# nkargas/Gen2-UHF-RFID-Reader

Measured on AMD Instinct MI355X. Metric: I/Q Msamples/s through matched_filter->gate->tag_decoder (+ EPC decodes/s), 40 kHz FM0, higher is better.
Workload: dtype f32; 1 GPU; configs[1]: batch of 1024 noise-replicas per GPU of the 71-round file_source_test stand-in trace, FM0 40 kHz BLF @ 2 Msps (1076066 raw I/Q samples each, sigma=0.002), generated and resident in HBM; streams_per_gpu=1024, hbm_bytes_traces=8815132672, parallelism=traces sharded per GPU, no collective

## Files before the change

gen2-uhf-rfid-reader_amd/csrc/rfid_capi.hip:

```cpp
#include <hip/hip_runtime.h>

#include <cmath>
#include <ctime>
#include <pthread.h>
#include <cstdio>
#include <cstdlib>
#include <cstring>
#include <deque>
#include <initializer_list>
#include <map>
#include <memory>
#include <new>
#include <vector>

#include "rfid_host_math.h"
#include "rfid_kernels.hpp"
#include "rfid_inventory.hpp"
#include "rfid_tracks.hpp"
#include "rfid_quality.hpp"
#include "rfid_repair.hpp"
#include "rfid_mi355x.h"
#include "rfid_gen2_host.h"
#define LS2_LAUNCH(kernel, gx, gy, block, args) \
  hipLaunchKernelGGL(rfidk::kernel, dim3((unsigned)(gx), (unsigned)(gy)), dim3((unsigned)(block)), 0, ls2_stream, args)
// ... 1689 lines not shown
  if (!c || !ms) return RFID_ERR_INVALID;
  return stage_ms(c, c->rep, ms);
}

int rfid_repair_window(rfid_ctx *c, const rfid_cf32 *gated, const rfid_decode_result *res, rfid_repair *out) {
  if (!c || !gated || !res || !out) return RFID_ERR_INVALID;
  if (res->type != RFID_DECODE_EPC) return fail(c, RFID_ERR_INVALID, "rfid_repair_window: not the result of an EPC window");
  HIPCHK(c, hipSetDevice(c->device));
  const size_t sz_w = up256(sizeof(float2) * (size_t)EPC_WIN), sz_r = up256(sizeof(rfid_decode_result));
  { int r = grow(c, c->rep_one, sz_w + sz_r + sizeof(rfid_repair)); if (r) return r; }
  char *b = (char *)c->rep_one.p;
  HIPCHK(c, hipMemcpyAsync(b, gated, sizeof(float2) * (size_t)EPC_WIN, hipMemcpyHostToDevice, c->stream));
  HIPCHK(c, hipMemcpyAsync(b + sz_w, res, sizeof(*res), hipMemcpyHostToDevice, c->stream));
  hipLaunchKernelGGL(repair_one_kernel, dim3(1), dim3(64), 0, c->stream, (const float2 *)b, (const rfid_decode_result *)(b + sz_w),
                     (rfid_repair *)(b + sz_w + sz_r));
  HIPCHK(c, hipGetLastError());
  HIPCHK(c, hipMemcpyAsync(out, b + sz_w + sz_r, sizeof(*out), hipMemcpyDeviceToHost, c->stream));
  HIPCHK(c, hipStreamSynchronize(c->stream));
  return RFID_OK;
}

}

namespace {

int pass_long_stream(rfid_ctx *c, const void *d_raw, int64_t raw_stride, int64_t n_raw, const void *d_lens, int want_scores) {
  HIPCHK(c, hipSetDevice(c->device));
  { int rj = join_tails(c); if (rj) return rj; }
  const int64_t n_out = n_raw / DECIM;
  const int64_t tiles = (n_out + MF_TILE - 1) / MF_TILE;
  int rc, enq = 0;
  bool ahead = false;
  if (raw_stride >= 2) {
    c->d_lens = (const int64_t *)d_lens;
    c->last_n_raw = n_raw;
    c->n_chunks_last = 0;
    ahead = c->alt.d_y != nullptr && c->ls2_ws_alt.p != nullptr && !c->alt_have && (c->knobs.overlap != 0);
    if (ahead && (rc = y_take_ahead(c))) return rc;
    HIPCHK_T(c, ev_mark(c, EV_MF_BEGIN, c->stream));
    HIPCHK_T(c, ev_mark(c, EV_MF_END, c->stream));
    LsOpts lo;
    lo.raw = d_raw; lo.raw_stride = raw_stride; lo.ahead = ahead;
    if ((rc = ls_enqueue(c, n_out, lo, &enq))) { c->y_touched = true; return rc; }
    if (!enq && ahead) {
      y_give_back(c);
      ahead = lo.ahead = false;
      if ((rc = ls_enqueue(c, n_out, lo, &enq))) return rc;
    }
  }
  if (enq) {
    c->fused_last = 2;
    MfFallbackArgs f;
    f.m = mf_args(c, d_raw, raw_stride, n_raw);
    f.skip_if = &c->d_ls2_ctl->ok; f.n_tiles = tiles;
    if ((rc = launch_mf_rows(c, c->stream, f, (tiles < 4096) ? tiles : 4096)) || (rc = rfid_batch_gate_impl(c, &c->d_ls2_ctl->ok)) ||
        (rc = rfid_batch_decode(c, want_scores)) || (rc = rfid_batch_stats(c))) { c->y_touched = true; return rc; }
    return y_pass_done(c, ahead);
  }
  c->y_touched = true;
  if ((rc = batch_mf_on(c, c->stream, d_raw, raw_stride, n_raw, d_lens))) return rc;
  LsOpts lo;
  if ((rc = ls_enqueue(c, n_out, lo, &enq))) return rc;
  if ((rc = rfid_batch_gate_impl(c, enq ? &c->d_ls2_ctl->ok : nullptr))) return rc;
  if ((rc = rfid_batch_decode(c, want_scores))) return rc;
  return rfid_batch_stats(c);
}

int pass_fused(rfid_ctx *c, const void *d_raw, int64_t raw_stride, int64_t n_raw, const void *d_lens, int want_scores) {
  HIPCHK(c, hipSetDevice(c->device));
  c->d_lens = (const int64_t *)d_lens;
  c->last_n_raw = n_raw;
  c->n_chunks_last = 0;
  const bool overlap = c->alt_have && !want_scores;
  { int rj = overlap ? set_take_next(c) : join_tails(c); if (rj) return rj; }
  HIPCHK(c, ev_mark(c, EV_MF_BEGIN, c->stream));
  HIPCHK(c, ev_mark(c, EV_MF_END, c->stream));
  HIPCHK(c, hipMemsetAsync(c->d_gstate, 0, sizeof(GateState) * (size_t)c->B, c->stream));
  HIPCHK(c, hipMemsetAsync(c->cur.d_flat_count, 0, 2 * sizeof(int), c->stream));
  GateArgs g = gate_args(c, n_raw / DECIM);
  g.y_w = c->cur.d_y;
  g.raw = (const float2 *)d_raw; g.raw_stride = raw_stride; g.n_raw = n_raw;
  g.raw_vec_ok = rows_vec_ok(d_raw, raw_stride);
  g.single_step = c->knobs.front_single_step;
  hipLaunchKernelGGL(front_end_fused_kernel, gate_grid(c), dim3(GATE_THREADS), 0, c->stream, g);
  HIPCHK(c, hipGetLastError());
  HIPCHK(c, ev_mark(c, EV_GATE_END, c->stream));
  c->fused_last = 1;
  if (overlap) return set_tails_on_stream2(c);
  int rc = rfid_batch_decode(c, want_scores);
  if (rc) return rc;
  return rfid_batch_stats(c);
}

int pass_chunked(rfid_ctx *c, const void *d_raw, int64_t raw_stride, int64_t n_raw, const void *d_lens, int want_scores) {
  const int nch = c->knobs.front_chunks;
  const int64_t tiles = (n_raw / DECIM + MF_TILE - 1) / MF_TILE;
  HIPCHK(c, hipSetDevice(c->device));
  { int rj = join_tails(c); if (rj) return rj; }
  if (!c->ev_mf[0]) {
    for (int i = 0; i <= rfid_ctx::MAX_CHUNKS; ++i) HIPCHK(c, hipEventCreate(&c->ev_mf[i]));
    for (int i = 0; i < 2 * rfid_ctx::MAX_CHUNKS; ++i) HIPCHK(c, hipEventCreate(&c->ev_gate[i]));
  }
  c->d_lens = (const int64_t *)d_lens;
  c->last_n_raw = n_raw;
  const int64_t tiles_per_chunk = (tiles + nch - 1) / nch;
  HIPCHK(c, hipEventRecord(c->ev_pass, c->stream));
  HIPCHK(c, hipStreamWaitEvent(c->stream2, c->ev_pass, 0));
  HIPCHK(c, hipMemsetAsync(c->d_gstate, 0, sizeof(GateState) * (size_t)c->B, c->stream2));
  HIPCHK(c, hipMemsetAsync(c->cur.d_flat_count, 0, 2 * sizeof(int), c->stream2));
  MfArgs m = mf_args(c, d_raw, raw_stride, n_raw);
  GateArgs g = gate_args(c, n_raw / DECIM);
  HIPCHK(c, ev_mark(c, EV_MF_BEGIN, c->stream));
  HIPCHK(c, hipEventRecord(c->ev_mf[0], c->stream));
  int used = 0;
  for (int k = 0; k < nch; ++k) {
    const int64_t t0 = (int64_t)k * tiles_per_chunk;
    if (t0 >= tiles) break;
    const int64_t tn = (t0 + tiles_per_chunk <= tiles) ? tiles_per_chunk : (tiles - t0);
    m.tile0 = t0;
    { int r = launch_mf_rows(c, c->stream, m, tn); if (r) return r; }
    HIPCHK(c, hipEventRecord(c->ev_mf[k + 1], c->stream));
    HIPCHK(c, hipStreamWaitEvent(c->stream2, c->ev_mf[k + 1], 0));
    g.pos0 = t0 * MF_TILE; g.chunk_len = tn * MF_TILE;
    HIPCHK(c, hipEventRecord(c->ev_gate[2 * k], c->stream2));
    hipLaunchKernelGGL(gate_scan_kernel, gate_grid(c), dim3(GATE_THREADS), 0, c->stream2, g);
    HIPCHK(c, hipGetLastError());
    HIPCHK(c, hipEventRecord(c->ev_gate[2 * k + 1], c->stream2));
    used = k + 1;
  }
  c->n_chunks_last = used;
  HIPCHK(c, hipEventRecord(c->ev_front_end, c->stream2));
  HIPCHK(c, hipStreamWaitEvent(c->stream, c->ev_front_end, 0));
  c->ev_valid[EV_MF_END] = false;
  HIPCHK(c, ev_mark(c, EV_GATE_END, c->stream));
  int rc = rfid_batch_decode(c, want_scores);
  if (rc) return rc;
  return rfid_batch_stats(c);
}

}

extern "C" {

int rfid_batch_process(rfid_ctx *c, const void *d_raw, int64_t raw_stride, int64_t n_raw, const void *d_lens,
                       int want_scores) {
  if (!c || !d_raw || n_raw < 0 || raw_stride < n_raw) return RFID_ERR_INVALID;
  if (!c->B) return RFID_ERR_STATE;
  if (n_raw > c->max_raw) return RFID_ERR_CAPACITY;
  ls_note_last_pass(c);
  const int64_t n_out = n_raw / DECIM;
  const int64_t tiles = (n_out + MF_TILE - 1) / MF_TILE;
  const int nch = c->knobs.front_chunks;
  if (nch < 2 && ls_applicable(c, c->B, n_out)) return pass_long_stream(c, d_raw, raw_stride, n_raw, d_lens, want_scores);
  c->d_ls2_ctl = nullptr;
  c->y_touched = true;
  if (nch < 2 && raw_stride >= 2 && !c->knobs.front_unfused) return pass_fused(c, d_raw, raw_stride, n_raw, d_lens, want_scores);
  c->fused_last = 0;
  if (tiles < 4 * (int64_t)nch || nch < 2) {
    int rc = rfid_batch_mf(c, d_raw, raw_stride, n_raw, d_lens);
    if (rc) return rc;
    if ((rc = rfid_batch_gate(c))) return rc;
    if ((rc = rfid_batch_decode(c, want_scores))) return rc;
    return rfid_batch_stats(c);
  }
  return pass_chunked(c, d_raw, raw_stride, n_raw, d_lens, want_scores);
}

// ... 605 lines not shown
```

gen2-uhf-rfid-reader_amd/csrc/rfid_kernels.hpp:

```cpp
#pragma once
#include <rfid_device_env.h>
#include "rfid_mi355x.h"

namespace rfidk {

constexpr int DECIM = 5;
constexpr int NTAPS = 25;
constexpr int WIN_LEN = 100;
constexpr int DC_LEN = 48;
constexpr int T1_SAMPLES = 96;
constexpr int PW_HALF = 2;
constexpr int GATE_N_SAT = 128;
static_assert(GATE_N_SAT > T1_SAMPLES && GATE_N_SAT > PW_HALF, "the saturated count must pass every comparison");
constexpr int NUM_PULSES_CMD = 5;
constexpr int RN16_WIN = 250;
constexpr int EPC_WIN = 1370;
constexpr int N_SYNC = 15;
constexpr int N_TCAND = 20;
constexpr float HALF_BIT = 5.0f;
constexpr float WIN_LEN_F = 100.0f;
constexpr float DC_LEN_F = 48.0f;
constexpr float THRESH_FRACTION = 0.75f;

constexpr int MF_TILE = 512;
// ... 248 lines not shown
    const int I = R - ((frac < 0.0f) ? 1 : 0);
    const uint64_t rodd = wv::ballot((R & 1) != 0) & ~tiemask;
    const uint64_t iodd = wv::ballot((I & 1) != 0) & tiemask;
    const uint64_t Q = prefix_xor64(rodd);
    const uint64_t gen = tiemask & Q, X = gen | ~tiemask;
    const uint64_t sum = X + gen + (uint64_t)(cb & 1u);
    const uint64_t W = X ^ gen ^ sum;
    const uint64_t par = (Q << 1) ^ W;
    const uint64_t up = (par ^ iodd) & tiemask;
    R = tie ? (I + (int)((up >> lane) & 1ull)) : R;
  }
  const uint32_t mag = (cb & 0x7fffffffu) + (uint32_t)wv::scan_add(R);
  const uint64_t badmask_s = wv::ballot(((mag ^ cb) & 0x7f800000u) != 0u) | wv::ballot((mag & 0x007fffffu) == 0u);
  const bool bad_c = e_b < 23u || e_b > 254u;
  out = wv::u2f(mag | sign);
  return (badmask_t | badmask_s) == 0ull && !bad_c;
}

RFID_DEVICE float chain_add_auto(float carry, float x, int lane) {
  float v;
  if (__builtin_expect(chain_add_scan(carry, x, lane, v), 1)) return v;
  return chain_add(carry, x, lane);
}

RFID_DEVICE uint64_t lane_range(int lo, int hi) {
  const uint64_t up = (hi >= 64) ? ~0ull : ((1ull << hi) - 1ull);
  const uint64_t dn = (lo >= 64) ? ~0ull : ((1ull << lo) - 1ull);
  return up & ~dn;
}

RFID_DEVICE void chain_add2(float cb, float xb, float cc, float xc, int lane, float &pb, float &pc) {
  const float b0 = (lane == 0) ? (cb + xb) : xb;
  const float c0 = (lane == 0) ? (cc + xc) : xc;
  pb = b0; pc = c0;
#pragma unroll
  for (int s = 1; s < 64; ++s) {
    pb = wv::shr1(pb) + b0;
    pc = wv::shr1(pc) + c0;
  }
}

struct GateRegs {
  float avg_c;
  int f_n, f_state, f_pulses, f_open, f_ung, f_type;
  int consumed;
  bool stop;
};

struct GateBackRegs {
  float dcr_c, dci_c;
  int dc_index;
  int run_closed;
  int ring_stale;
  float2 prev_yv;
  int win_seq, n_complete, written;
  int pos0, strm;
};

struct GateSlot {
  float amp[64];
  float d[64];
  alignas(16) int b_word;
  int b_pad0_;
  uint64_t b_closedmask;
  uint64_t b_openmask;
  int b_pad1_[2];
  float2 yv[64];
  float tre[64];
  float tim[64];
  int spec_bad;
  int pad_[3];
};

RFID_DEVICE void gate_spec_dc(GateSlot &slot, float2 yv, float2 &prev_yv, int lane) {
  const int src = (lane < DC_LEN) ? (lane + 64 - DC_LEN) : (lane - DC_LEN);
  const float pre = wv::shfl(prev_yv.x, src), pim = wv::shfl(prev_yv.y, src);
  const float cre = wv::shfl(yv.x, src), cim = wv::shfl(yv.y, src);
  const float ore = (lane < DC_LEN) ? pre : cre, oim = (lane < DC_LEN) ? pim : cim;
  const float nr = yv.x - ore, ni = yv.y - oim;
  slot.tre[lane] = div_const_fast<DC_LEN>(nr);
  slot.tim[lane] = div_const_fast<DC_LEN>(ni);
  slot.spec_bad = ((div_const_bad(nr) | div_const_bad(ni)) != 0ull) ? 1 : 0;
  prev_yv = yv;
}

RFID_DEVICE void gate_produce(GateSlot &slot, float2 yv_in, int pos, int n, int lane,
                              float *lds_win, int &win_index) {
  const int nvalid = (n - pos < 64) ? (n - pos) : 64;
  const bool valid = lane < nvalid;
  const float2 yv = valid ? yv_in : make_float2(0.0f, 0.0f);
  const float amp = wv::hypot_f(yv.x, yv.y);
  int wi = win_index + lane;
  if (wi >= WIN_LEN) wi -= WIN_LEN;
  const float amp_old = lds_win[wi];
  const float nd = valid ? (amp - amp_old) : 0.0f;
  wv::wave_sync();
  if (valid) lds_win[wi] = amp;
  wv::wave_sync();
  win_index += nvalid;
  if (win_index >= WIN_LEN) win_index -= WIN_LEN;
  const float d = div_const<WIN_LEN>(nd);
  slot.amp[lane] = amp;
  slot.d[lane] = d;
}

RFID_DEVICE void gate_record_window(const GateArgs &a, GateBackRegs &g, int ol, int wtype, int pos, int n, int s,
                                    int lane, float dcr, float dci) {
  const float odr = wv::readlane(dcr, ol), odi = wv::readlane(dci, ol);
  const int wlen = wtype ? EPC_WIN : RN16_WIN;
  const int start = g.pos0 + pos + ol;
  if (a.mode == 0 && start + wlen <= n) {
    if (lane == 0 && g.win_seq < a.wmax) {
      rfid_window w;
      w.stream = g.strm; w.seq = g.win_seq; w.start = start; w.type = wtype;
      w.dc_re = odr; w.dc_im = odi;
      a.wtab[(int64_t)s * a.wmax + g.win_seq] = w;
    }
    g.n_complete++;
  }
  g.win_seq++;
}

RFID_DEVICE void gate_flat_lists(const GateArgs &a, int s, int first, int cnt, int lane) {
  if (!a.flat || cnt <= 0) return;
  wv::global_release();
  const rfid_window *row = a.wtab + (int64_t)s * a.wmax;
  const uint64_t lt = (lane == 0) ? 0ull : (~0ull >> (64 - lane));
  int n1 = 0;
  for (int j0 = 0; j0 < cnt; j0 += 64) {
    const int j = j0 + lane;
    const int ty = (j < cnt) ? wv::load_coherent_i32(&row[first + j].type) : 0;
    n1 += wv::popc64(wv::ballot(ty != 0));
  }
  int base = 0;
  if (lane < 2) {
    const int want = lane ? n1 : (cnt - n1);
    if (want > 0) base = wv::atomic_add(a.flat_count + lane, want);
  }
  const int base0 = wv::readlane(base, 0), base1 = wv::readlane(base, 1);
  int done0 = 0, done1 = 0;
  for (int j0 = 0; j0 < cnt; j0 += 64) {
    const int j = j0 + lane;
    rfid_window w;
    w.type = 0;
    if (j < cnt) w = wv::load_coherent_window(&row[first + j]);
    const uint64_t m1 = wv::ballot(j < cnt && w.type != 0), m0 = wv::ballot(j < cnt && w.type == 0);
    if (j < cnt) {
      const int slotw = w.type ? (base1 + done1 + wv::popc64(m1 & lt)) : (base0 + done0 + wv::popc64(m0 & lt));
      if (slotw < a.flat_cap) a.flat[(int64_t)(w.type ? 1 : 0) * a.flat_cap + slotw] = w;
    }
    done0 += wv::popc64(m0); done1 += wv::popc64(m1);
  }
}

RFID_DEVICE void gate_fsm_step(const int mode, GateRegs &g, const uint64_t below, const uint64_t above, const int pos, int &nvalid,
                               uint64_t &closedmask, uint64_t &openmask, int &open_lane, int &open_type) {
  const bool plain_open = (nvalid == 64) && g.f_open && (g.f_ung - g.f_n > 64);
  const bool plain_closed = (nvalid == 64) && !g.f_open && (g.f_state == 1) && (below == 0) &&
                            !((g.f_pulses > NUM_PULSES_CMD) && (T1_SAMPLES - g.f_n < 64));
  closedmask = 0; openmask = 0;
  open_lane = 0xff; open_type = 0;

  if (__builtin_expect(plain_open || plain_closed, 1)) {
    g.f_n += 64;
    closedmask = plain_closed ? ~0ull : 0ull;
    openmask = plain_closed ? 0ull : ~0ull;
// ... 290 lines not shown
  int stop;
  int fsm_done;
  int prod_done;
};

struct GateRawRegs {
  float4 v[GATE_RAW_LD];
};

struct GateTrue { static constexpr bool value = true; };
struct GateFalse { static constexpr bool value = false; };
template <bool INTERIOR = false>
RFID_DEVICE void gate_load_raw(GateRawRegs &r, const float2 *xs, int64_t hi_idx, int64_t r0, int lane, bool vec) {
  const float2 *p = xs + r0;
  if (INTERIOR) {
    const char *pb = reinterpret_cast<const char *>(p);
#pragma unroll
    for (int j = 0; j < GATE_RAW_LD; ++j) {
      int q = lane + 64 * j;
      q = (q < GATE_RAW4) ? q : (GATE_RAW4 - 1);
      r.v[j] = *reinterpret_cast<const float4 *>(pb + (uint32_t)(16 * q));
    }
    return;
  }
  const int lo = (r0 < 0) ? (int)(-r0) : 0;
  int64_t hrel = hi_idx - r0;
  hrel = (hrel > (1 << 30)) ? (1 << 30) : hrel;
  hrel = (hrel < -(1 << 30)) ? -(1 << 30) : hrel;
  const int hi = (int)hrel;
#pragma unroll
  for (int j = 0; j < GATE_RAW_LD; ++j) {
    int q = lane + 64 * j;
    q = (q < GATE_RAW4) ? q : (GATE_RAW4 - 1);
    int ri = 2 * q;
    ri = (ri < lo) ? lo : ri;
    ri = (ri > hi) ? hi : ri;
    if (vec) {
      r.v[j] = *reinterpret_cast<const float4 *>(p + ri);
    } else {
      const float2 lo2 = p[ri], hi2 = p[ri + 1];
      r.v[j] = make_float4(lo2.x, lo2.y, hi2.x, hi2.y);
    }
  }
}

RFID_DEVICE float2 gate_fir_step(const GateRawRegs &r, float4 *tile4, int lane, bool first) {
  wv::wave_sync();
#pragma unroll
  for (int j = 0; j < GATE_RAW_LD; ++j) {
    const int q = lane + 64 * j;
    float4 v = r.v[j];
    if (j == 0 && first && q < (NTAPS - 1) / 2) v = make_float4(0.0f, 0.0f, 0.0f, 0.0f);
    tile4[q] = v;
  }
  wv::wave_sync();
  const float2 *tile = reinterpret_cast<const float2 *>(tile4);
  static_assert(NTAPS == 25, "lds_sum25_in_order");
  return wv::lds_sum25_in_order(&tile[DECIM * lane]);
}

RFID_DEVICE GateShared *gate_shared() {
  RFID_SHARED GateShared sh_all[GATE_STREAMS_PER_WG];
  return sh_all;
}

struct GateExtent { int n_total, n, nsteps; };
RFID_DEVICE GateExtent gate_extent(const GateArgs &a, int strm) {
  int64_t n64 = a.n_dec;
  if (a.lens) {
    int64_t r = a.lens[strm];
    if (r < 0) r = 0;
    n64 = r / DECIM;
    if (n64 > a.n_dec) n64 = a.n_dec;
  }
  GateExtent e;
  e.n_total = wv::uniform((int)n64);
  int64_t nl = n64 - a.pos0;
  if (nl > a.chunk_len) nl = a.chunk_len;
  if (nl < 0) nl = 0;
  e.n = wv::uniform((int)nl);
  e.nsteps = (e.n + 63) >> 6;
  return e;
}
RFID_DEVICE void gate_filter_tail(GateShared &sh, const float2 *xs, int64_t hi_idx, int64_t rbase, bool vec, float2 *yw, int k0,
                                  int nsteps, int n, bool at_start, int &back_seen, float2 &prev_yv, int lane) {
  for (int k = k0; k < nsteps; ++k) {
    while (k - back_seen >= GATE_SLOTS) { back_seen = wv::lds_load(&sh.back_seq); if (k - back_seen >= GATE_SLOTS) wv::backoff(); }
    GateRawRegs r;
    gate_load_raw(r, xs, hi_idx, rbase + (int64_t)k * 64 * DECIM, lane, vec);
    float2 yv = gate_fir_step(r, sh.rawtile, lane, k == 0 && at_start);
    if (64 * k + lane < n) yw[64 * k + lane] = yv;
    else yv = make_float2(0.0f, 0.0f);
    sh.slots[k % GATE_SLOTS].yv[lane] = yv;
    gate_spec_dc(sh.slots[k % GATE_SLOTS], yv, prev_yv, lane);
    wv::lds_store(&sh.fir_seq, k + 1, lane);
  }
}
RFID_DEVICE void gate_back_begin(GateBackRegs &g, const GateState *st, float2 *lds_dc, int64_t pos0, int strm, int lane) {
  if (lane < DC_LEN) lds_dc[lane] = make_float2(st->dcr_re[lane], st->dcr_im[lane]);
  g.dcr_c = wv::uniform(st->dc_re); g.dci_c = wv::uniform(st->dc_im);
  g.dc_index = wv::uniform(st->dc_index);
  g.run_closed = 0; g.ring_stale = 0;
  g.prev_yv = make_float2(0.0f, 0.0f);
  g.win_seq = wv::uniform(st->win_seq);
  g.n_complete = 0; g.written = 0;
  g.pos0 = (int)pos0; g.strm = strm;
  wv::wave_sync();
}
RFID_DEVICE void gate_back_end(const GateArgs &a, GateBackRegs &g, GateState *st, float2 *lds_dc, int row, int64_t pos0, int lane) {
  if (g.ring_stale) {
    if (lane >= 64 - DC_LEN) {
      int di = g.dc_index + (lane - (64 - DC_LEN));
      if (di >= DC_LEN) di -= DC_LEN;
      lds_dc[di] = g.prev_yv;
    }
    wv::wave_sync();
  }
  if (lane < DC_LEN) { st->dcr_re[lane] = lds_dc[lane].x; st->dcr_im[lane] = lds_dc[lane].y; }
  if (lane == 0) {
    st->dc_re = g.dcr_c; st->dc_im = g.dci_c; st->win_seq = g.win_seq; st->dc_index = g.dc_index;
    if (a.mode != 0) a.io[1] = g.written;
  }
  if (a.mode == 0) {
    const int before = (pos0 > 0) ? wv::uniform(a.wcount[row]) : 0;
    int tot = before + g.n_complete;
    tot = (tot < a.wmax) ? tot : a.wmax;
    if (lane == 0) a.wcount[row] = tot;
    gate_flat_lists(a, row, before, tot - before, lane);
  }
}
RFID_DEVICE void gate_fsm_begin(GateRegs &g, const GateState *st, int n) {
  g.avg_c = wv::uniform(st->avg_ampl);
  g.f_n = wv::uniform(st->n_samples); g.f_state = wv::uniform(st->signal_state);
  g.f_pulses = wv::uniform(st->num_pulses); g.f_open = wv::uniform(st->gate_open);
  g.f_ung = wv::uniform(st->n_to_ungate); g.f_type = wv::uniform(st->wtype);
  if (g.f_ung == 0) g.f_ung = g.f_type ? EPC_WIN : RN16_WIN;
  g.consumed = n; g.stop = false;
}
template <bool FUSED>
RFID_DEVICE void gate_fsm_end(const GateArgs &a, const GateRegs &g, GateState *st, GateShared &sh, const float2 *ys, int win_index0, int lane) {
  while (wv::lds_load(&sh.prod_done) == 0) wv::backoff();
  {
    const int c = g.consumed;
    const int first = (c > WIN_LEN) ? (c - WIN_LEN) : 0;
    for (int i = first + lane; i < c; i += 64) {
      const float2 v = FUSED ? wv::load_coherent(&ys[i]) : ys[i];
      st->win[(win_index0 + i) % WIN_LEN] = wv::hypot_f(v.x, v.y);
    }
  }
  if (lane == 0) {
    st->avg_ampl = g.avg_c;
    st->n_samples = g.f_n; st->signal_state = g.f_state; st->num_pulses = g.f_pulses;
    st->gate_open = g.f_open; st->n_to_ungate = g.f_ung; st->wtype = g.f_type;
    st->win_index = (win_index0 + g.consumed) % WIN_LEN;
    if (a.mode != 0) a.io[0] = g.consumed;
  }
}

template <bool FUSED>
RFID_DEVICE void gate_scan_body(const GateArgs &a) {
  GateShared *sh_all = gate_shared();
  const int lane = wv::lane_id();
  const int wave = wv::uniform((int)(threadIdx.x >> 6));
  const int role = wave / GATE_STREAMS_PER_WG;
  const int sl = wave % GATE_STREAMS_PER_WG;
  const int s = (int)blockIdx.x * GATE_STREAMS_PER_WG + sl;
  GateShared &sh = sh_all[sl];
  if (lane == 0 && role == 0) {
    sh.fir_seq = 0; sh.prod_seq = 0; sh.fsm_seq = 0; sh.back_seq = 0; sh.stop = 0; sh.fsm_done = 0; sh.prod_done = 0;
  }
  wv::block_sync();
  if (s >= a.n_streams) return;
  if (a.skip_if && wv::uniform(*a.skip_if) != 0) return;
  const int strm = s, row = s;
  const int64_t pos0 = a.pos0;
  GateState *st = a.state + row;
  const float2 *ys = a.y + (int64_t)strm * a.y_stride + pos0;
// ... 213 lines not shown
  lds_win[wi1] = amp1;
  wv::wave_sync();
  static_assert(WIN_LEN == 100, "128 mod WIN_LEN");
  win_index += 128 - WIN_LEN;
  if (win_index >= WIN_LEN) win_index -= WIN_LEN;
  const float nd0 = amp0 - old0, nd1 = amp1 - old1;
  float d0, d1;
  if (__builtin_expect((div_const_bad(nd0) | div_const_bad(nd1)) == 0ull, 1)) {
    d0 = div_const_fast<WIN_LEN>(nd0); d1 = div_const_fast<WIN_LEN>(nd1);
  } else {
    d0 = wv::fdiv(nd0, (float)WIN_LEN); d1 = wv::fdiv(nd1, (float)WIN_LEN);
  }
  s0.amp[lane] = amp0; s0.d[lane] = d0;
  s1.amp[lane] = amp1; s1.d[lane] = d1;
}

struct GateNextPair {
  int step;
  int sq;
  float amp0, d0, amp1, d1;
};
RFID_DEVICE void gate_fetch_pair(GateNextPair &nx, const int *seq, const GateSlot *s0, const GateSlot *s1, int k, int lane) {
  wv::compiler_fence();
  nx.sq = wv::lds_peek(seq);
  wv::compiler_fence();
  nx.amp0 = s0->amp[lane]; nx.d0 = s0->d[lane];
  nx.amp1 = s1->amp[lane]; nx.d1 = s1->d[lane];
  wv::compiler_fence();
  nx.step = k;
}
RFID_DEVICE void gate_consume_pair(GateRegs &g, GateSlot *s0, GateSlot *s1, const GateSlot *n0, const GateSlot *n1,
                                   GateNextPair &nx, const int *seq, int k, int lane) {
  if (!(nx.step == k && wv::uniform(nx.sq) > k + 1)) {
    while (wv::lds_load(seq) <= k + 1) wv::backoff();
    gate_fetch_pair(nx, seq, s0, s1, k, lane);
  }
  const float f_amp0 = nx.amp0, f_d0 = nx.d0, f_amp1 = nx.amp1, f_d1 = nx.d1;
  float avg0, avg1;
  if (__builtin_expect(!chain_add_scan_pair(g.avg_c, f_d0, f_d1, lane, avg0, avg1), 0)) {
    avg0 = chain_add_auto(g.avg_c, f_d0, lane);
    avg1 = chain_add_auto(wv::readlane(avg0, 63), f_d1, lane);
  }
  g.avg_c = wv::readlane(avg1, 63);
  const float th0 = avg0 * THRESH_FRACTION, th1 = avg1 * THRESH_FRACTION;
  const uint64_t below0 = wv::ballot(f_amp0 < th0), below1 = wv::ballot(f_amp1 < th1);
  gate_fetch_pair(nx, seq, n0, n1, k + 2, lane);
  uint64_t closed0, open0, closed1, open1;
  int ol0 = 0xff, ot0 = 0, ol1 = 0xff, ot1 = 0;
  const bool plain_open = g.f_open && (g.f_ung - g.f_n > 128);
  const bool plain_closed = !g.f_open && (g.f_state == 1) && ((below0 | below1) == 0) &&
                            !((g.f_pulses > NUM_PULSES_CMD) && (T1_SAMPLES - g.f_n < 128));
  if (__builtin_expect(plain_open || plain_closed, 1)) {
    g.f_n += 128;
    closed0 = closed1 = plain_closed ? ~0ull : 0ull;
    open0 = open1 = plain_closed ? 0ull : ~0ull;
    if (!g.f_open && g.f_n > GATE_N_SAT) g.f_n = GATE_N_SAT;
  } else {
    const uint64_t above0 = wv::ballot(f_amp0 > th0), above1 = wv::ballot(f_amp1 > th1);
    int nv = 64;
    gate_fsm_step(0, g, below0, above0, 64 * k, nv, closed0, open0, ol0, ot0);
    nv = 64;
    gate_fsm_step(0, g, below1, above1, 64 * k + 64, nv, closed1, open1, ol1, ot1);
  }
  wv::lds_store_rec(&s0->b_word, ((closed0 != 0) ? 1 : 0) | ((open0 != 0) ? 4 : 0) | (64 << 8) | (ol0 << 16) | (ot0 << 24), closed0, lane);
  wv::lds_store_rec(&s1->b_word, ((closed1 != 0) ? 1 : 0) | ((open1 != 0) ? 4 : 0) | (64 << 8) | (ol1 << 16) | (ot1 << 24), closed1, lane);
}

RFID_DEVICE void gate_back_pair(const GateArgs &a, GateBackRegs &g, const GateSlot *s0, const GateSlot *s1, int pos, int n_total,
                                int row, int lane, float2 *lds_dc, float2 *lds_tmp) {
  int word0, word1;
  uint64_t closed0, closed1;
  const int sb0 = wv::lds_peek(&s0->spec_bad), sb1 = wv::lds_peek(&s1->spec_bad);
  wv::lds_load_rec(&s0->b_word, word0, closed0);
  wv::lds_load_rec(&s1->b_word, word1, closed1);
  if (((word0 | word1) & 1) == 0) {
    g.run_closed = 0;
    return;
  }
  bool stop;
  gate_back_desc(a, g, s0, word0, closed0, (word0 & 4) ? 1ull : 0ull, sb0, pos, n_total, row, lane, lds_dc, lds_tmp, stop);
  gate_back_desc(a, g, s1, word1, closed1, (word1 & 4) ? 1ull : 0ull, sb1, pos + 64, n_total, row, lane, lds_dc, lds_tmp, stop);
}

RFID_DEVICE void gate_pairs_body(const GateArgs &a) {
  GateShared *sh_all = gate_shared();
  const int lane = wv::lane_id();
  const int wave = wv::uniform((int)(threadIdx.x >> 6));
  const int role = wave / GATE_STREAMS_PER_WG;
  const int sl = wave % GATE_STREAMS_PER_WG;
  const int s = (int)blockIdx.x * GATE_STREAMS_PER_WG + sl;
  GateShared &sh = sh_all[sl];
  if (lane == 0 && role == 0) {
    sh.fir_seq = 0; sh.prod_seq = 0; sh.fsm_seq = 0; sh.back_seq = 0; sh.stop = 0; sh.fsm_done = 0; sh.prod_done = 0;
  }
  wv::block_sync();
  if (s >= a.n_streams) return;
  if (a.skip_if && wv::uniform(*a.skip_if) != 0) return;
  const int strm = s, row = s;
  const int64_t pos0 = a.pos0;
  GateState *st = a.state + row;
  const float2 *ys = a.y + (int64_t)strm * a.y_stride + pos0;
  const GateExtent ex = gate_extent(a, strm);
  const int n_total = ex.n_total, n = ex.n, nsteps = ex.nsteps;
  const int nfull = n >> 6;
  const int npaired = nfull & ~1;
  const int win_index0 = wv::uniform(st->win_index);

  if (role == 1) {
    float2 prev_yv = make_float2(0.0f, 0.0f);
    const float2 *xs = a.raw + (int64_t)strm * a.raw_stride;
    const bool vec = a.raw_vec_ok != 0;
    const int64_t hi_idx = vec ? ((a.raw_stride - 2) & ~(int64_t)1) : (a.raw_stride - 2);
    float2 *yw = a.y_w + (int64_t)strm * a.y_stride + pos0;
    const int64_t rbase = pos0 * DECIM - (NTAPS - 1);
    static_assert(GATE_RAW_DEPTH % 2 == 0 && GATE_SLOTS % 2 == 0, "a group is whole pairs, a pair does not straddle the ring's wrap");
    const int ngroups = nfull / GATE_RAW_DEPTH;
    const bool at_start = pos0 == 0;
    int back_seen = 0;
    if (ngroups > 0) {
      GateRawRegs buf[GATE_RAW_DEPTH];
#pragma unroll
      for (int u = 0; u < GATE_RAW_DEPTH; ++u) {
        gate_load_raw(buf[u], xs, hi_idx, rbase + (int64_t)u * 64 * DECIM, lane, vec);
        wv::compiler_fence();
      }
      int g_fast = 0;
      if (vec) {
        const int64_t j_max = (hi_idx - 2 * (GATE_RAW4 - 1) - rbase) / (64 * DECIM);
        int64_t gf = (j_max + 1) / GATE_RAW_DEPTH - 1;
        gf = (gf < 0) ? 0 : gf;
        g_fast = (gf > ngroups) ? ngroups : (int)gf;
      }
      auto group = [&](int grp, auto interior) {
#pragma unroll
        for (int u = 0; u < GATE_RAW_DEPTH; ++u) {
          const int k = grp * GATE_RAW_DEPTH + u;
          if ((u & 1) == 0)
            while (k + 1 - back_seen >= GATE_SLOTS) { back_seen = wv::lds_load(&sh.back_seq); if (k + 1 - back_seen >= GATE_SLOTS) wv::backoff(); }
          const float2 yv = gate_fir_step(buf[u], sh.rawtile, lane, u == 0 && grp == 0 && at_start);
          gate_load_raw<decltype(interior)::value>(buf[u], xs, hi_idx, rbase + (int64_t)(k + GATE_RAW_DEPTH) * 64 * DECIM, lane, vec);
          yw[64 * k + lane] = yv;
          sh.slots[k % GATE_SLOTS].yv[lane] = yv;
          gate_spec_dc(sh.slots[k % GATE_SLOTS], yv, prev_yv, lane);
          if ((u & 1) == 1) wv::lds_store(&sh.fir_seq, k + 1, lane);
        }
      };
      int grp = 0;
      for (; grp < g_fast; ++grp) group(grp, GateTrue());
      for (; grp < ngroups; ++grp) group(grp, GateFalse());
    }
    gate_filter_tail(sh, xs, hi_idx, rbase, vec, yw, ngroups * GATE_RAW_DEPTH, nsteps, n, at_start, back_seen, prev_yv, lane);
    wv::global_release();
    wv::lds_store(&sh.prod_done, 1, lane);
  } else if (role == 3) {
    for (int j = lane; j < WIN_LEN; j += 64) sh.win[j] = st->win[j];
    int win_index = win_index0;
    wv::wave_sync();
    int fir_seen = 0;
    int k = 0;
    for (; k < npaired; k += 2) {
      while (fir_seen <= k + 1) { fir_seen = wv::lds_load(&sh.fir_seq); if (fir_seen <= k + 1) wv::backoff(); }
      GateSlot &s0 = sh.slots[k % GATE_SLOTS], &s1 = sh.slots[k % GATE_SLOTS + 1];
      gate_produce_pair(s0, s1, s0.yv[lane], s1.yv[lane], lane, sh.win, win_index);
      wv::lds_store(&sh.prod_seq, k + 2, lane);
    }
    for (; k < nsteps; ++k) {
      while (fir_seen <= k) { fir_seen = wv::lds_load(&sh.fir_seq); if (fir_seen <= k) wv::backoff(); }
      GateSlot &slot = sh.slots[k % GATE_SLOTS];
      gate_produce(slot, slot.yv[lane], 64 * k, n, lane, sh.win, win_index);
      wv::lds_store(&sh.prod_seq, k + 1, lane);
    }
  } else if (role == 2) {
    float2 *lds_dc = sh.dc, *lds_tmp = sh.tmp;
    GateBackRegs g;
    gate_back_begin(g, st, lds_dc, pos0, strm, lane);
    int fsm_seen = 0;
    int k = 0;
    for (; k < npaired; k += 2) {
      while (fsm_seen <= k + 1) { fsm_seen = wv::lds_load(&sh.fsm_seq); if (fsm_seen <= k + 1) wv::backoff(); }
      gate_back_pair(a, g, &sh.slots[k % GATE_SLOTS], &sh.slots[k % GATE_SLOTS + 1], 64 * k, n_total, row, lane, lds_dc, lds_tmp);
      wv::lds_store(&sh.back_seq, k + 2, lane);
    }
    for (; k < nsteps; ++k) {
      while (fsm_seen <= k) { fsm_seen = wv::lds_load(&sh.fsm_seq); if (fsm_seen <= k) wv::backoff(); }
      bool stop;
      gate_back(a, g, &sh.slots[k % GATE_SLOTS], 64 * k, n_total, row, lane, lds_dc, lds_tmp, stop);
      wv::lds_store(&sh.back_seq, k + 1, lane);
    }
    gate_back_end(a, g, st, lds_dc, row, pos0, lane);
  } else {
    wv::set_priority_high();
    GateRegs g;
    gate_fsm_begin(g, st, n);
    int k = 0;
    {
      GateNextPair nx;
      nx.step = -1; nx.sq = 0; nx.amp0 = nx.d0 = nx.amp1 = nx.d1 = 0.0f;
      for (; k < npaired; k += 2) {
        GateSlot *s0 = &sh.slots[k % GATE_SLOTS], *n0 = &sh.slots[(k + 2) % GATE_SLOTS];
        gate_consume_pair(g, s0, s0 + 1, n0, n0 + 1, nx, &sh.prod_seq, k, lane);
        wv::lds_store(&sh.fsm_seq, k + 2, lane);
      }
    }
    GateNext nx;
    nx.step = -1; nx.sq = 0; nx.amp = nx.d = 0.0f;
    for (; k < nsteps; ++k) {
      gate_consume(a, g, &sh.slots[k % GATE_SLOTS], &sh.slots[(k + 1) % GATE_SLOTS], nx, &sh.prod_seq, k, 64 * k, n, lane);
      wv::lds_store(&sh.fsm_seq, k + 1, lane);
      wv::lds_prefetch_wait<2>(nx.sq, nx.amp, nx.d);
    }
    wv::lds_store(&sh.fsm_done, 1, lane);
    gate_fsm_end<true>(a, g, st, sh, ys, win_index0, lane);
  }
}

RFID_KERNEL_OCC(GATE_THREADS, GATE_WAVES_PER_SIMD) void gate_scan_kernel(GateArgs a) { gate_scan_body<false>(a); }
RFID_KERNEL_OCC(GATE_THREADS, GATE_WAVES_PER_SIMD) void front_end_fused_kernel(GateArgs a) {
  if (a.single_step == 0 && a.mode == 0) gate_pairs_body(a);
  else gate_scan_body<true>(a);
}

constexpr int LS_QUIET = EPC_WIN + T1_SAMPLES + 1 + WIN_LEN + DC_LEN;
static_assert(GATE_N_SAT < WIN_LEN + DC_LEN - 1, "n_samples must have saturated at every cut (147 samples after a window at least)");

struct LsCutArgs {
  const float2 *y;
  int64_t y_stride;
  const int64_t *lens;
  int64_t n_dec;
  int chunk;
  int limit;
  int max_b;
  int quiet;
  int *cut;
};

RFID_DEVICE void ls_cut_body(const LsCutArgs &a, const int s, const int j) {
  const int lane = wv::lane_id();
  int64_t n64 = a.n_dec;
  if (a.lens) { int64_t r = a.lens[s]; if (r < 0) r = 0; n64 = r / DECIM; if (n64 > a.n_dec) n64 = a.n_dec; }
  const int n = (int)n64;
  const int P = j * a.chunk;
  int *out = a.cut + (int64_t)s * a.max_b + j;
  if (P >= n) { if (lane == 0) *out = -1; return; }
  const float2 *ys = a.y + (int64_t)s * a.y_stride;
  int lo = P - a.quiet - 64;
  if (lo < 0) lo = 0;
  float ref = 0.0f;
  for (int base = lo; base < P; base += 64) {
    const int i = base + lane;
    float m2 = 0.0f;
    if (i < P) { const float2 v = ys[i]; m2 = v.x * v.x + v.y * v.y; }
    ref = (m2 > ref) ? m2 : ref;
  }
#pragma unroll
  for (int off = 32; off >= 1; off >>= 1) { const float o = wv::shfl_xor(ref, off); ref = (o > ref) ? o : ref; }
  const float theta = 0.7225f * ref;
  int run = 0, found = -1;
  int end = P + a.limit;
  if (end > n) end = n;
  const uint64_t lt = (lane == 0) ? 0ull : (~0ull >> (64 - lane));
  for (int base = lo; base < end && found < 0; base += 64) {
    const int i = base + lane;
    bool low = false;
    if (i < n) { const float2 v = ys[i]; low = (v.x * v.x + v.y * v.y) < theta; } else low = true;
    const uint64_t lowmask = wv::ballot(low);
    const uint64_t below = lowmask & lt;
    const int q = below ? (lane - 1 - (63 - __builtin_clzll(below))) : (run + lane);
    const uint64_t hit = wv::ballot(i >= P && i < end && q >= a.quiet);
    if (hit) found = base + wv::ffs64(hit);
    run = lowmask ? __builtin_clzll(lowmask) : (run + 64);
  }
  if (lane == 0) *out = found;
}
RFID_KERNEL(64) void ls_cut_kernel(LsCutArgs a) { ls_cut_body(a, (int)blockIdx.y, (int)blockIdx.x + 1); }
struct LsCut2Args { LsCutArgs a, b; int n_streams; };
RFID_KERNEL(64) void ls_cut2_kernel(LsCut2Args p) {
  const int y = (int)blockIdx.y, j = (int)blockIdx.x + 1;
  if (y < p.n_streams) { if (j < p.a.max_b) ls_cut_body(p.a, y, j); }
  else if (j < p.b.max_b) ls_cut_body(p.b, y - p.n_streams, j);
}

struct GatedPack {
  const rfid_window *wtab; const int *wcount; const rfid_decode_result *res; int wmax;
  const float2 *y;
  char *pack;
  int n_hdr, usual;
  const int *only_if;
};
constexpr int GATED_HDR = 64;
RFID_DEVICE size_t gated_pack_hdr_bytes(int n_hdr) { return (size_t)GATED_HDR + (sizeof(rfid_window) + sizeof(rfid_decode_result)) * (size_t)n_hdr; }
RFID_KERNEL(256) void gated_windows_kernel(GatedPack a) {
  int n = *a.wcount;
  if (a.only_if && *a.only_if == 0) n = 0;
  const int b = (int)blockIdx.x;
  char *pk = a.pack;
  rfid_window *hw = reinterpret_cast<rfid_window *>(pk + GATED_HDR);
  rfid_decode_result *hr = reinterpret_cast<rfid_decode_result *>(hw + a.n_hdr);
  if (b == 0 && threadIdx.x == 0) *reinterpret_cast<int *>(pk) = n;
  if (n > a.wmax) n = a.wmax;
  if (b >= n) return;
  if (b < a.n_hdr && threadIdx.x == 0) { hw[b] = a.wtab[b]; hr[b] = a.res[b]; }
// ... 949 lines not shown
```

Baseline: 462,300 Msamples/s.

## Split fused front-end kernel and read DC-lag samples from LDS slots

The fused front-end kernel previously carried both the paired gate body and the scan body, so one kernel had to budget registers for both paths. This change adds a separate single-step kernel chosen on the host and leaves the fused kernel with only the paired path. Inside that path, the DC-removal lag now reads the previous and current yv values from LDS slots at a precomputed byte offset, replacing four wave shuffles and the prev_yv register copy. The cost is an extra wave_sync and LDS traffic per step, plus a dependence on the previous slot still being intact in the ring, and the kernel forces mode to 0.

```diff
diff --git a/gen2-uhf-rfid-reader_amd/csrc/rfid_capi.hip b/gen2-uhf-rfid-reader_amd/csrc/rfid_capi.hip
--- a/gen2-uhf-rfid-reader_amd/csrc/rfid_capi.hip
+++ b/gen2-uhf-rfid-reader_amd/csrc/rfid_capi.hip
@@ -1795,7 +1795,8 @@
   g.raw = (const float2 *)d_raw; g.raw_stride = raw_stride; g.n_raw = n_raw;
   g.raw_vec_ok = rows_vec_ok(d_raw, raw_stride);
   g.single_step = c->knobs.front_single_step;
-  hipLaunchKernelGGL(front_end_fused_kernel, gate_grid(c), dim3(GATE_THREADS), 0, c->stream, g);
+  if (g.single_step) hipLaunchKernelGGL(front_end_fused_single_kernel, gate_grid(c), dim3(GATE_THREADS), 0, c->stream, g);
+  else hipLaunchKernelGGL(front_end_fused_kernel, gate_grid(c), dim3(GATE_THREADS), 0, c->stream, g);
   HIPCHK(c, hipGetLastError());
   HIPCHK(c, ev_mark(c, EV_GATE_END, c->stream));
   c->fused_last = 1;
diff --git a/gen2-uhf-rfid-reader_amd/csrc/rfid_kernels.hpp b/gen2-uhf-rfid-reader_amd/csrc/rfid_kernels.hpp
--- a/gen2-uhf-rfid-reader_amd/csrc/rfid_kernels.hpp
+++ b/gen2-uhf-rfid-reader_amd/csrc/rfid_kernels.hpp
@@ -354,6 +354,16 @@
   slot.tim[lane] = div_const_fast<DC_LEN>(ni);
   slot.spec_bad = ((div_const_bad(nr) | div_const_bad(ni)) != 0ull) ? 1 : 0;
   prev_yv = yv;
+}
+
+RFID_DEVICE void gate_spec_dc_lds(GateSlot &slot, const GateSlot &prev, float2 yv, int src8, int lane) {
+  wv::wave_sync();
+  const char *base = reinterpret_cast<const char *>((lane < DC_LEN) ? prev.yv : slot.yv);
+  const float2 o = *reinterpret_cast<const float2 *>(base + src8);
+  const float nr = yv.x - o.x, ni = yv.y - o.y;
+  slot.tre[lane] = div_const_fast<DC_LEN>(nr);
+  slot.tim[lane] = div_const_fast<DC_LEN>(ni);
+  slot.spec_bad = ((div_const_bad(nr) | div_const_bad(ni)) != 0ull) ? 1 : 0;
 }
 
 RFID_DEVICE void gate_produce(GateSlot &slot, float2 yv_in, int pos, int n, int lane,
@@ -810,8 +820,9 @@
   e.nsteps = (e.n + 63) >> 6;
   return e;
 }
+template <bool SPEC_LDS = false>
 RFID_DEVICE void gate_filter_tail(GateShared &sh, const float2 *xs, int64_t hi_idx, int64_t rbase, bool vec, float2 *yw, int k0,
-                                  int nsteps, int n, bool at_start, int &back_seen, float2 &prev_yv, int lane) {
+                                  int nsteps, int n, bool at_start, int &back_seen, float2 &prev_yv, int lane, int src8 = 0) {
   for (int k = k0; k < nsteps; ++k) {
     while (k - back_seen >= GATE_SLOTS) { back_seen = wv::lds_load(&sh.back_seq); if (k - back_seen >= GATE_SLOTS) wv::backoff(); }
     GateRawRegs r;
@@ -820,7 +831,8 @@
     if (64 * k + lane < n) yw[64 * k + lane] = yv;
     else yv = make_float2(0.0f, 0.0f);
     sh.slots[k % GATE_SLOTS].yv[lane] = yv;
-    gate_spec_dc(sh.slots[k % GATE_SLOTS], yv, prev_yv, lane);
+    if (SPEC_LDS) gate_spec_dc_lds(sh.slots[k % GATE_SLOTS], sh.slots[(k + GATE_SLOTS - 1) % GATE_SLOTS], yv, src8, lane);
+    else gate_spec_dc(sh.slots[k % GATE_SLOTS], yv, prev_yv, lane);
     wv::lds_store(&sh.fir_seq, k + 1, lane);
   }
 }
@@ -1200,10 +1212,12 @@
   gate_back_desc(a, g, s1, word1, closed1, (word1 & 4) ? 1ull : 0ull, sb1, pos + 64, n_total, row, lane, lds_dc, lds_tmp, stop);
 }
 
-RFID_DEVICE void gate_pairs_body(const GateArgs &a) {
+RFID_DEVICE void gate_pairs_body(const GateArgs &a_in) {
+  GateArgs a = a_in;
+  a.mode = 0;
   GateShared *sh_all = gate_shared();
-  const int lane = wv::lane_id();
   const int wave = wv::uniform((int)(threadIdx.x >> 6));
+  const int lane = (int)threadIdx.x - 64 * wave;
   const int role = wave / GATE_STREAMS_PER_WG;
   const int sl = wave % GATE_STREAMS_PER_WG;
   const int s = (int)blockIdx.x * GATE_STREAMS_PER_WG + sl;
@@ -1226,6 +1240,8 @@
 
   if (role == 1) {
     float2 prev_yv = make_float2(0.0f, 0.0f);
+    const int src8 = 8 * ((lane < DC_LEN) ? (lane + 64 - DC_LEN) : (lane - DC_LEN));
+    sh.slots[GATE_SLOTS - 1].yv[lane] = make_float2(0.0f, 0.0f);
     const float2 *xs = a.raw + (int64_t)strm * a.raw_stride;
     const bool vec = a.raw_vec_ok != 0;
     const int64_t hi_idx = vec ? ((a.raw_stride - 2) & ~(int64_t)1) : (a.raw_stride - 2);
@@ -1259,7 +1275,7 @@
           gate_load_raw<decltype(interior)::value>(buf[u], xs, hi_idx, rbase + (int64_t)(k + GATE_RAW_DEPTH) * 64 * DECIM, lane, vec);
           yw[64 * k + lane] = yv;
           sh.slots[k % GATE_SLOTS].yv[lane] = yv;
-          gate_spec_dc(sh.slots[k % GATE_SLOTS], yv, prev_yv, lane);
+          gate_spec_dc_lds(sh.slots[k % GATE_SLOTS], sh.slots[(k + GATE_SLOTS - 1) % GATE_SLOTS], yv, src8, lane);
           if ((u & 1) == 1) wv::lds_store(&sh.fir_seq, k + 1, lane);
         }
       };
@@ -1267,7 +1283,7 @@
       for (; grp < g_fast; ++grp) group(grp, GateTrue());
       for (; grp < ngroups; ++grp) group(grp, GateFalse());
     }
-    gate_filter_tail(sh, xs, hi_idx, rbase, vec, yw, ngroups * GATE_RAW_DEPTH, nsteps, n, at_start, back_seen, prev_yv, lane);
+    gate_filter_tail<true>(sh, xs, hi_idx, rbase, vec, yw, ngroups * GATE_RAW_DEPTH, nsteps, n, at_start, back_seen, prev_yv, lane, src8);
     wv::global_release();
     wv::lds_store(&sh.prod_done, 1, lane);
   } else if (role == 3) {
@@ -1333,9 +1349,12 @@
 }
 
 RFID_KERNEL_OCC(GATE_THREADS, GATE_WAVES_PER_SIMD) void gate_scan_kernel(GateArgs a) { gate_scan_body<false>(a); }
+RFID_KERNEL_OCC(GATE_THREADS, GATE_WAVES_PER_SIMD) void front_end_fused_single_kernel(GateArgs a) { gate_scan_body<true>(a); }
 RFID_KERNEL_OCC(GATE_THREADS, GATE_WAVES_PER_SIMD) void front_end_fused_kernel(GateArgs a) {
-  if (a.single_step == 0 && a.mode == 0) gate_pairs_body(a);
-  else gate_scan_body<true>(a);
+#if !defined(__HIPCC__)
+  if (a.single_step != 0 || a.mode != 0) { front_end_fused_single_kernel(a); return; }
+#endif
+  gate_pairs_body(a);
 }
 
 constexpr int LS_QUIET = EPC_WIN + T1_SAMPLES + 1 + WIN_LEN + DC_LEN;
```

Result: no change. 465,700 Msamples/s (median of 6 runs) (+0.7%).
